# strasdat/ScaViSLAM

Hardware: AMD Instinct MI355X
Metric: stereo frames/sec + DWO Schur ms @ 50 KF / 20k pts (higher is better)
Workload: dtype u8/int32 (FAST, ZNSSD), f32+f64 (dense tracking), f64 (Schur); 1 GPU

## Files before the change

scavislam_amd/csrc/dense.hip:

```cpp
#include "common.h"
#include "lm6.h"
#include "seqsum.h"
#include <algorithm>

namespace {

constexpr int NSUM = 28;

struct Acc {
  double v[NSUM];
  long long n;
  __device__ __forceinline__ void zero() {
#pragma unroll
    for (int i = 0; i < NSUM; ++i) v[i] = 0;
    n = 0;
  }
};

template <class P>
__device__ __forceinline__ float interp32f(P m, int stride, float u, float v) {
  float x = floorf(u), y = floorf(v);
  float sx = u - x, sy = v - y;
  float wx0 = 1 - sx, wx1 = sx, wy0 = 1 - sy, wy1 = sy;
  int xi = (int)x, yi = (int)y;
  const P p = m + (unsigned)(yi * stride + xi);
  float v00 = p[0], v10 = p[1], v01 = p[stride], v11 = p[stride + 1];
  return (wx0 * wy0) * v00 + (wx0 * wy1) * v01 + (wx1 * wy0) * v10 + (wx1 * wy1) * v11;
}

struct LevelArgs {
  const float *cloud; const uint8_t *prev; const float *cur, *dx, *dy;
  int pstride, fstride;
  svs_cam cam;
  const uint8_t *cur8;
  int c8stride;
};

#define SVS_AS1 __attribute__((address_space(1)))
typedef float svs_f4 __attribute__((ext_vector_type(4)));
struct LevelArgsG {
  const SVS_AS1 float *cloud; const SVS_AS1 uint8_t *prev; const SVS_AS1 float *cur, *dx, *dy;
  int pstride, fstride;
  svs_cam cam;
  const SVS_AS1 uint8_t *cur8;
  int c8stride;
};
__device__ __forceinline__ float4 load_f4(const float *p) { return *reinterpret_cast<const float4 *>(p); }
__device__ __forceinline__ float4 load_f4(const SVS_AS1 float *p) { const svs_f4 v = *(const SVS_AS1 svs_f4 *)p; return make_float4(v.x, v.y, v.z, v.w); }
__device__ __forceinline__ uint32_t load_u32_unaligned(const uint8_t *p) { uint32_t w; __builtin_memcpy(&w, p, 4); return w; }
__device__ __forceinline__ uint32_t load_u32_unaligned(const SVS_AS1 uint8_t *p) {
  typedef uint32_t u32_unaligned __attribute__((aligned(1)));
  return *(const SVS_AS1 u32_unaligned *)p;
}

template <class P>
__device__ __forceinline__ void taps_u8(P img, int stride, float u, float v, float &ic, float &gx, float &gy) {
  const float sc = (float)(1. / 255.);
  const float x = floorf(u), y = floorf(v);
  const float sx = u - x, sy = v - y;
  const float wx0 = 1 - sx, wx1 = sx, wy0 = 1 - sy, wy1 = sy;
  const int xi = (int)x, yi = (int)y;
  float f[4][4];
  const unsigned o0 = (unsigned)((yi - 1) * stride + (xi - 1));
#pragma unroll
  for (int r = 0; r < 4; ++r) {
    const uint32_t w4 = load_u32_unaligned(img + (o0 + (unsigned)(r * stride)));
#pragma unroll
    for (int c = 0; c < 4; ++c) f[r][c] = (float)((w4 >> (8 * c)) & 0xff) * sc;
  }
  const float w00 = wx0 * wy0, w01 = wx0 * wy1, w10 = wx1 * wy0, w11 = wx1 * wy1;
  ic = w00 * f[1][1] + w01 * f[2][1] + w10 * f[1][2] + w11 * f[2][2];
  gx = w00 * (f[1][2] - f[1][0]) + w01 * (f[2][2] - f[2][0]) + w10 * (f[1][3] - f[1][1]) + w11 * (f[2][3] - f[2][1]);
  gy = w00 * (f[2][1] - f[0][1]) + w01 * (f[3][1] - f[1][1]) + w10 * (f[2][2] - f[0][2]) + w11 * (f[3][2] - f[1][2]);
}

struct SampleIn { float4 c4; uint8_t prev; };
template <class LA>
__device__ __forceinline__ SampleIn sample_load(const LA &L, int u, int v, int cw, bool in_range) {
  SampleIn s;
  s.c4 = in_range ? load_f4(L.cloud + 4u * (unsigned)(v * cw + u)) : make_float4(0.f, 0.f, 1.f, -1.f);
  s.prev = L.prev[(unsigned)(((in_range ? v : 0) * 4) * L.pstride + (in_range ? u : 0) * 4)];
  return s;
}
__device__ __forceinline__ double rcp_rn(double b) {
  double r = __builtin_amdgcn_rcp(b);
  double e = __builtin_fma(-b, r, 1.0);
  r = __builtin_fma(e, r, r);
  e = __builtin_fma(-b, r, 1.0);
  return __builtin_fma(e, r, r);
}
__device__ __forceinline__ double div_rn(double a, double b, double r) {
  const double q = a * r;
  return __builtin_fma(__builtin_fma(-q, b, a), r, q);
}

template <bool JAC, bool U8SRC = false, int TM = 0, class LA = LevelArgs>
__device__ __forceinline__ void sample_cpu_sem(const LA &L, const double *T, const SampleIn &in, bool in_range, Acc &a,
                                               const float *ip_lut = nullptr, float *term_out = nullptr) {
  const float4 c4 = in.c4;
  bool ok = in_range && (c4.w > 0);
  const double xp0 = c4.x, xp1 = c4.y, xp2 = c4.z;
  const double x = T[0] * xp0 + T[1] * xp1 + T[2] * xp2 + T[3];
  const double y = T[4] * xp0 + T[5] * xp1 + T[6] * xp2 + T[7];
  const double z = T[8] * xp0 + T[9] * xp1 + T[10] * xp2 + T[11];
  const double rz = rcp_rn(z);
  float uvx = (float)(L.cam.f * div_rn(x, z, rz) + L.cam.cx);
  float uvy = (float)(L.cam.f * div_rn(y, z, rz) + L.cam.cy);
  ok = ok && (fabsf(uvx) < 1e9f && fabsf(uvy) < 1e9f);
  const int ui = ok ? (int)uvx : 0, vi = ok ? (int)uvy : 0;
  ok = ok && (ui >= 2 && vi >= 2 && ui < L.cam.w - 2 && vi < L.cam.h - 2);
  if (!ok) { uvx = 2.f; uvy = 2.f; }
  const float ip = ip_lut ? ip_lut[in.prev] : (float)((1. / 255.) * in.prev);
  float ic, g8x = 0.f, g8y = 0.f;
  if (U8SRC) taps_u8(L.cur8, L.c8stride, uvx, uvy, ic, g8x, g8y);
  else ic = interp32f(L.cur, L.fstride, uvx, uvy);
  float res = ip - ic;
  res = fminf(fmaxf(res, -0.1f), 0.1f);
  if (!ok) res = 0.f;
  a.v[27] += (double)(res * res);
  if constexpr (TM != 0) *term_out = res * res;
  a.n += ok ? 1 : 0;
  if (JAC) {
    const float gx = ok ? (float)(0.5 * (U8SRC ? g8x : interp32f(L.dx, L.fstride, uvx, uvy))) : 0.f;
    const float gy = ok ? (float)(0.5 * (U8SRC ? g8y : interp32f(L.dy, L.fstride, uvx, uvy))) : 0.f;
    const double zs = ok ? z : 1.0, xs = ok ? x : 0.0, ys = ok ? y : 0.0;
    {
      const double f = L.cam.f, iz = ok ? rz : 1.0, iz2 = iz * iz, fx = f * iz, xz = xs * iz2 * f, yz = ys * iz2 * f;
      const double r0[6] = {-fx, 0, xz, xz * ys, -__builtin_fma(xz, xs, f), ys * fx};
      const double r1[6] = {0, -fx, yz, __builtin_fma(yz, ys, f), -(yz * xs), -(xs * fx)};
      double J[6];
      J[0] = gx * r0[0];
      J[1] = gy * r1[1];
#pragma unroll
      for (int k = 2; k < 6; ++k) J[k] = __builtin_fma(gx, r0[k], gy * r1[k]);
      int k = 0;
#pragma unroll
      for (int c = 0; c < 6; ++c)
#pragma unroll
        for (int r = 0; r <= c; ++r) { a.v[k] = __builtin_fma(J[r], J[c], a.v[k]); ++k; }
#pragma unroll
      for (int i = 0; i < 6; ++i) a.v[21 + i] = __builtin_fma(J[i], (double)res, a.v[21 + i]);
    }
  }
}

template <int NWAVES>
__device__ __forceinline__ void block_reduce(Acc &a, double (*s_part)[NSUM + 1], double *out_vals ) {
  const int lane = threadIdx.x & 63, wave = threadIdx.x >> 6;
  double x[32];
#pragma unroll
  for (int i = 0; i < NSUM; ++i) x[i] = a.v[i];
  x[NSUM] = (double)a.n;
#pragma unroll
  for (int i = NSUM + 1; i < 32; ++i) x[i] = 0.0;
#pragma unroll
  for (int step = 0; step < 5; ++step) {
    const int half = 16 >> step, bit = 1 << step;
    const bool up = (lane & bit) != 0;
#pragma unroll
    for (int k = 0; k < half; ++k) {
      const double send = up ? x[k] : x[k + half];
      const double keep = up ? x[k + half] : x[k];
      x[k] = keep + __shfl_xor(send, bit, 64);
    }
  }
  x[0] += __shfl_xor(x[0], 32, 64);
  const int idx = ((lane & 1) << 4) | ((lane & 2) << 2) | (lane & 4) | ((lane & 8) >> 2) | ((lane & 16) >> 4);
  if (lane < 32 && idx <= NSUM) s_part[wave][idx] = x[0];
  __syncthreads();
  if (threadIdx.x <= NSUM) {
    double s = 0;
    for (int w = 0; w < NWAVES; ++w) s += s_part[w][threadIdx.x];
    out_vals[threadIdx.x] = s;
  }
  __syncthreads();
}

template <bool JAC>
__global__ __launch_bounds__(256) void dense_pass_cpu_sem_kernel(LevelArgs L, size_t cloud_b, size_t prev_b, size_t f_b,
                                                                 const double *__restrict__ Tarr, double *__restrict__ partials) {
  __shared__ double s_part[4][NSUM + 1];
  __shared__ double s_out[NSUM + 1];
  const int slot = blockIdx.y;
  L.cloud += slot * cloud_b; L.prev += slot * prev_b; L.cur += slot * f_b; L.dx += slot * f_b; L.dy += slot * f_b;
  double T[12];
#pragma unroll
  for (int i = 0; i < 12; ++i) T[i] = Tarr[(size_t)slot * 12 + i];
  const int cw = L.cam.w / 4, ch = L.cam.h / 4, n = cw * ch;
  Acc a;
  a.zero();
  for (int i = blockIdx.x * 256 + threadIdx.x; i < n; i += gridDim.x * 256) sample_cpu_sem<JAC>(L, T, sample_load(L, i % cw, i / cw, cw, true), true, a);
  block_reduce<4>(a, s_part, s_out);
  if (threadIdx.x <= NSUM) partials[((size_t)slot * gridDim.x + blockIdx.x) * (NSUM + 1) + threadIdx.x] = s_out[threadIdx.x];
}

__global__ void dense_finalize_kernel(const double *__restrict__ partials, int nblocks, svs_dense_sums *__restrict__ out) {
  const int slot = blockIdx.x, t = threadIdx.x;
  if (t > NSUM) return;
  double s = 0;
  for (int b = 0; b < nblocks; ++b) s += partials[((size_t)slot * nblocks + b) * (NSUM + 1) + t];
  svs_dense_sums *o = &out[slot];
  if (t < 21) o->H[t] = s;
  else if (t < 27) o->b[t - 21] = s;
  else if (t == 27) o->chi2 = (double)(float)s;
  else o->n_valid = (long long)s;
}

struct TrackArgs {
  LevelArgs lv[3];
  size_t cloud_b[3], prev_b[3], f_b[3], c8_b[3];
  double *T_jac;
  svs_dense_lm_record *rec; int rec_cap; int32_t *n_rec;
};

constexpr int TRK_THREADS = 512;
constexpr int TRK_MINW_BIG = 4;
constexpr int TRK_UNROLL = 1;
constexpr bool TRK_T_SCALAR = true;

template <bool JAC, bool U8SRC, int TM = 0, class LA = LevelArgs>
__device__ __forceinline__ void track_pass(const LA &L, const double *T_in, double (*s_part)[NSUM + 1], double *s_out, const float *ip_lut,
                                           int first, int nwg, float *t_buf = nullptr) {
  const int cw = L.cam.w / 4, ch = L.cam.h / 4, n = cw * ch;
  double T[12];
#pragma unroll
  for (int i = 0; i < 12; ++i)
    T[i] = TRK_T_SCALAR ? __hiloint2double(__builtin_amdgcn_readfirstlane(__double2hiint(T_in[i])), __builtin_amdgcn_readfirstlane(__double2loint(T_in[i]))) : T_in[i];
  Acc a;
  a.zero();
  const int STEP = TRK_UNROLL * TRK_THREADS * nwg;
  const int su = STEP % cw, sv = STEP / cw;
  SampleIn nxt[TRK_UNROLL];
  int pu[TRK_UNROLL], pv[TRK_UNROLL];
#pragma unroll
  for (int q = 0; q < TRK_UNROLL; ++q) {
    const int j = first + q * TRK_THREADS * nwg;
    pu[q] = j % cw; pv[q] = j / cw;
    const bool in = pv[q] < ch;
    nxt[q] = sample_load(L, in ? pu[q] : 0, in ? pv[q] : 0, cw, in);
  }
  typedef __attribute__((address_space(1))) float *gptr_t;
  static_assert(TM == 0 || TRK_UNROLL == 1, "the deferred term store keeps one term per lane");
  float pend_t = 0.f;
  gptr_t pend_p = (gptr_t)t_buf + first - STEP;
  bool pend = false;
  auto flush = [&]() {
    if constexpr (TM == 1) { if (pend) *pend_p = pend_t; }
    if constexpr (TM == 2) { if (pend) __hip_atomic_store(pend_p, pend_t, __ATOMIC_RELAXED, __HIP_MEMORY_SCOPE_AGENT); }
  };
  for (int i = first; i < n; i += STEP) {
    if constexpr (TM != 0) { flush(); pend_p += STEP; pend = t_buf != nullptr; }
    SampleIn cur[TRK_UNROLL];
#pragma unroll
    for (int q = 0; q < TRK_UNROLL; ++q) {
      cur[q] = nxt[q];
      pu[q] += su; pv[q] += sv;
      if (pu[q] >= cw) { pu[q] -= cw; ++pv[q]; }
      const bool in = pv[q] < ch;
      nxt[q] = sample_load(L, in ? pu[q] : 0, in ? pv[q] : 0, cw, in);
    }
#pragma unroll
    for (int q = 0; q < TRK_UNROLL; ++q) {
      if constexpr (TM != 0) sample_cpu_sem<JAC, U8SRC, TM, LA>(L, T, cur[q], true, a, ip_lut, &pend_t);
      else sample_cpu_sem<JAC, U8SRC, 0, LA>(L, T, cur[q], i + q * TRK_THREADS * nwg < n, a, ip_lut);
    }
  }
  if constexpr (TM != 0) flush();
  block_reduce<TRK_THREADS / 64>(a, s_part, s_out);
}

struct PassArgs { LevelArgs L; double T[12]; float *t_buf; int wg, nwg; };
__shared__ PassArgs g_pa;
__shared__ double g_s_part[TRK_THREADS / 64][NSUM + 1];
__shared__ double g_s_out[NSUM + 1];
__shared__ float g_iplut[256];
__device__ __forceinline__ int uni_i32(int v) { return __builtin_amdgcn_readfirstlane(v); }
__device__ __forceinline__ double uni_f64(double v) { return __hiloint2double(__builtin_amdgcn_readfirstlane(__double2hiint(v)), __builtin_amdgcn_readfirstlane(__double2loint(v))); }
template <class T>
__device__ __forceinline__ T *uni_ptr(T *p) {
  const unsigned long long u = (unsigned long long)p;
  const unsigned lo = __builtin_amdgcn_readfirstlane((unsigned)u), hi = __builtin_amdgcn_readfirstlane((unsigned)(u >> 32));
  return (T *)(((unsigned long long)hi << 32) | lo);
}
template <bool U8SRC, int TM>
__device__ __forceinline__ void track_pass_from_lds() {
  LevelArgsG L;
  L.cloud = (const SVS_AS1 float *)uni_ptr(g_pa.L.cloud); L.prev = (const SVS_AS1 uint8_t *)uni_ptr(g_pa.L.prev);
  L.cur = (const SVS_AS1 float *)uni_ptr(g_pa.L.cur); L.dx = (const SVS_AS1 float *)uni_ptr(g_pa.L.dx); L.dy = (const SVS_AS1 float *)uni_ptr(g_pa.L.dy);
  L.cur8 = (const SVS_AS1 uint8_t *)uni_ptr(g_pa.L.cur8);
  L.pstride = uni_i32(g_pa.L.pstride); L.fstride = uni_i32(g_pa.L.fstride); L.c8stride = uni_i32(g_pa.L.c8stride);
  L.cam.f = uni_f64(g_pa.L.cam.f); L.cam.cx = uni_f64(g_pa.L.cam.cx); L.cam.cy = uni_f64(g_pa.L.cam.cy); L.cam.b = 0;
  L.cam.w = uni_i32(g_pa.L.cam.w); L.cam.h = uni_i32(g_pa.L.cam.h);
  const int nwg = uni_i32(g_pa.nwg), first = uni_i32(g_pa.wg) * TRK_THREADS + (int)threadIdx.x;
  track_pass<true, U8SRC, TM, LevelArgsG>(L, g_pa.T, g_s_part, g_s_out, g_iplut, first, nwg, uni_ptr(g_pa.t_buf));
}
template <bool U8SRC, int TM>
__device__ __noinline__ void track_pass_call() { track_pass_from_lds<U8SRC, TM>(); }

typedef const __attribute__((address_space(1))) float *svs_gptr_f32;
typedef const __attribute__((address_space(1))) svs_f4 *svs_gptr_f4;
template <bool COH, typename P>
__device__ __forceinline__ float seq_term_load(P p) {
  if constexpr (COH) return __hip_atomic_load(p, __ATOMIC_RELAXED, __HIP_MEMORY_SCOPE_AGENT); else return *p;
}
template <bool COH = false, typename P = const float *>
__device__ __forceinline__ float seq_sum_f32(P t, int n) {
  float acc = 0.f;
  const int lane = threadIdx.x & 63;
  for (int base = 0; base < n; base += 64) {
    const float v = base + lane < n ? seq_term_load<COH, P>(t + base + lane) : 0.f;
#pragma unroll
    for (int l = 0; l < 64; ++l) acc = acc + __builtin_bit_cast(float, __builtin_amdgcn_readlane(__builtin_bit_cast(int, v), l));
  }
  return acc;
}
__device__ __forceinline__ float seq_chi2_f32(const float *t, int n) {
  __shared__ float s_seq;
  __syncthreads();
  if (threadIdx.x < 64) { const float v = seq_sum_f32(t, n); if (threadIdx.x == 0) s_seq = v; }
  __syncthreads();
  return s_seq;
}

constexpr int SEQ_Q = TRK_THREADS >= 512 ? 10 : 13;
constexpr int SEQ_RUN_MAX = 4 * SEQ_Q;
constexpr int SEQ_STAGE_FLOATS = 48 * SEQ_RUN_MAX;
struct SeqShared {
  SvsSeqMap pref[TRK_THREADS];
  unsigned char eb[TRK_THREADS];
  short slot[TRK_THREADS];
  unsigned long long unsafe[TRK_THREADS / 64];
  double wave_P[TRK_THREADS / 64];
  int wave_c[TRK_THREADS / 64], wave_u[TRK_THREADS / 64];
  float stage[SEQ_STAGE_FLOATS];
  float result;
  int fell_back;
};
template <bool COH>
__device__ __forceinline__ void seq_load_run(svs_gptr_f32 p, int nq, svs_f4 (&v)[SEQ_Q]) {
  if constexpr (COH) {
    static_assert(SEQ_Q == 10 || SEQ_Q == 13, "the blocks below issue ten (+ three) loads");
    asm volatile("global_load_dwordx4 %0, %10, off sc1\n\t"
                 "global_load_dwordx4 %1, %10, off offset:16 sc1\n\t"
                 "global_load_dwordx4 %2, %10, off offset:32 sc1\n\t"
                 "global_load_dwordx4 %3, %10, off offset:48 sc1\n\t"
                 "global_load_dwordx4 %4, %10, off offset:64 sc1\n\t"
                 "global_load_dwordx4 %5, %10, off offset:80 sc1\n\t"
                 "global_load_dwordx4 %6, %10, off offset:96 sc1\n\t"
                 "global_load_dwordx4 %7, %10, off offset:112 sc1\n\t"
                 "global_load_dwordx4 %8, %10, off offset:128 sc1\n\t"
                 "global_load_dwordx4 %9, %10, off offset:144 sc1\n\t"
                 "s_waitcnt vmcnt(0)"
                 : "=&v"(v[0]), "=&v"(v[1]), "=&v"(v[2]), "=&v"(v[3]), "=&v"(v[4]), "=&v"(v[5]), "=&v"(v[6]), "=&v"(v[7]), "=&v"(v[8]), "=&v"(v[9])
                 : "v"(p)
                 : "memory");
    if constexpr (SEQ_Q == 13)
      asm volatile("global_load_dwordx4 %0, %3, off offset:160 sc1\n\t"
                   "global_load_dwordx4 %1, %3, off offset:176 sc1\n\t"
                   "global_load_dwordx4 %2, %3, off offset:192 sc1\n\t"
                   "s_waitcnt vmcnt(0)"
                   : "=&v"(v[SEQ_Q - 3]), "=&v"(v[SEQ_Q - 2]), "=&v"(v[SEQ_Q - 1])
                   : "v"(p)
                   : "memory");
  } else {
#pragma unroll
    for (int q = 0; q < SEQ_Q; ++q) v[q] = q < nq ? *reinterpret_cast<svs_gptr_f4>(p + 4 * q) : svs_f4{0.f, 0.f, 0.f, 0.f};
  }
}
__shared__ SeqShared g_seq_sh;
template <bool COH>
__device__ __noinline__ float exact_seq_sum_f32(const float *t_flat, int n) {
  SeqShared &sh = g_seq_sh;
  svs_gptr_f32 t = (svs_gptr_f32)t_flat;
  const int tid = threadIdx.x, lane = tid & 63, wave = tid >> 6;
  const int S = max(4, (div_up(n, TRK_THREADS) + 3) & ~3);
  if (S > SEQ_RUN_MAX) {
    __syncthreads();
    if (wave == 0) { const float v = seq_sum_f32<COH, svs_gptr_f32>(t, n); if (lane == 0) { sh.result = v; sh.fell_back = 1; } }
    __syncthreads();
    return sh.result;
  }
  const int nq = S / 4;
  const int j0 = min(n, tid * S), j1 = min(n, j0 + S);
  const bool empty = j0 >= j1;
  svs_f4 v[SEQ_Q];
  seq_load_run<COH>(t + (empty ? 0 : j0), nq, v);
  double ps = 0;
  int cnt = 0;
#pragma unroll
  for (int q = 0; q < SEQ_Q; ++q)
#pragma unroll
    for (int c = 0; c < 4; ++c) {
      if (!(q < nq && j0 + 4 * q + c < j1)) v[q][c] = 0.f;
      ps += (double)v[q][c];
      cnt += v[q][c] != 0.f ? 1 : 0;
    }
  double incl = ps;
  int cincl = cnt;
#pragma unroll
  for (int d = 1; d < 64; d <<= 1) {
    const double o = __shfl_up(incl, d, 64);
    const int oc = __shfl_up(cincl, d, 64);
    if (lane >= d) { incl += o; cincl += oc; }
  }
// ... 441 lines not shown
    int level;
    if (!resume) {
      track_pass_from_lds<U8SRC, TM>();
      if constexpr (MULTI) { all_workgroups(); if (s_failed) { failed = true; break; } }
      level = g_ts.level;
      const int phase = g_ts.phase, cur = g_ts.cur, n_rec = g_ts.n_rec;
      const int n_lvl = (A.lv[level].cam.w / 4) * (A.lv[level].cam.h / 4);
      if (phase == 0) {
        const double S = g_s_out[27];
        const float chi2 = (float)S;
        __syncthreads();
        if (tid < 27) g_sH[tid] = g_s_out[tid];
        if (tid == 0) {
          g_ts.S_old = S; g_ts.nv_old = (int)g_s_out[NSUM]; g_ts.chi2 = chi2; g_ts.seq_old_ok = 0; g_ts.seq_old = 0.f;
          ++g_ts.passes; ++g_ts.n_rec; g_ts.work16 += 16 >> (2 * level);
          if (A.rec && wg == 0 && n_rec < A.rec_cap) A.rec[(size_t)slot * A.rec_cap + n_rec] = svs_dense_lm_record{level, 2, chi2, chi2};
        }
      } else {
        const double S_old = g_ts.S_old, S_new = g_s_out[27];
        const int nv_old = g_ts.nv_old, nv_new = (int)g_s_out[NSUM];
        float seq_old = g_ts.seq_old;
        bool seq_old_ok = g_ts.seq_old_ok != 0;
        unsigned n_exact = 0;
        const TrkVerdict V = track_accept<MULTI>(G, slot, S_old, S_new, nv_old, nv_new, tb0, cur, n_lvl, true, wg, nwg, g_ts.chi2, seq_old, seq_old_ok, n_decisions, n_old_sums, n_exact);
        if (V.failed) { if (tid == 0) s_failed = true; failed = true; break; }
        const bool accept = V.accept;
        const float chi2 = V.chi2, new_chi2 = V.new_chi2;
        double mx = -1;
        for (int q = 0; q < 6; ++q) mx = fmax(mx, fabs(g_sx[q]));
        const int it = g_ts.it + 1;
        level_done = !accept || mx <= 1e-10 || it >= 15;
        __syncthreads();
        if (accept) {
          if (tid < 12) g_sT[tid] = g_sTn[tid];
          if (tid < 27) g_sH[tid] = g_s_out[tid];
        }
        if (tid == 0) {
          if (accept) { g_ts.S_old = S_new; g_ts.nv_old = nv_new; g_ts.cur = cur ^ 1; g_ts.chi2 = new_chi2; }
          g_ts.seq_old = seq_old; g_ts.seq_old_ok = seq_old_ok ? 1 : 0; g_ts.it = it; g_ts.n_exact += n_exact;
          ++g_ts.passes; ++g_ts.n_rec; g_ts.work16 += 16 >> (2 * level);
          if (A.rec && wg == 0 && n_rec < A.rec_cap) A.rec[(size_t)slot * A.rec_cap + n_rec] = svs_dense_lm_record{level, accept ? 1 : 0, chi2, new_chi2};
        }
        if constexpr (!MULTI) {
          if (!level_done && level == 0 && C.K >= 0 && it >= C.K) parked = true;
        }
      }
      __syncthreads();
      if (parked) break;
    } else {
      resume = false;
      level = g_ts.level;
    }
    if (level_done) {
      if (level == 0) break;
      if (tid == 0) enter_level(level - 1);
      if (tid >= 64 && tid < 76) g_pa.T[tid - 64] = g_sT[tid - 64];
    } else {
      if (tid >= 64 && tid < 76) g_sTj[level][tid - 64] = g_sT[tid - 64];
      if (tid < 64) track_solve_call();
      __syncthreads();
      if (tid < 12) g_pa.T[tid] = g_sTn[tid];
      if (tid == 12) { g_pa.t_buf = tb0 ? tb0 + (size_t)(g_ts.cur ^ 1) * G.terms_b : nullptr; g_ts.phase = 1; }
    }
    __syncthreads();
  }
  if constexpr (!MULTI) {
    if (parked) {
      TrkPark &P = C.park[slot];
      if (tid == 0) { P.ts = g_ts; C.list[atomicAdd(C.count, 1u)] = slot; }
      if (tid < 12) P.T[tid] = g_sT[tid];
      if (tid >= 64 && tid < 64 + 27) P.H[tid - 64] = g_sH[tid - 64];
      if (tid >= 128 && tid < 128 + 36) P.Tj[tid - 128] = g_sTj[(tid - 128) / 12][(tid - 128) % 12];
      return;
    }
  }
  if (wg != 0) return;
  if (failed) { if (tid == 0 && passes_out) passes_out[slot] = -1; return; }
  if (tid < 12) T_io[(size_t)slot * 12 + tid] = g_sT[tid];
  if (tid == 0 && passes_out) passes_out[slot] = g_ts.passes;
  if (tid == 0 && A.n_rec) A.n_rec[slot] = g_ts.n_rec;
  if (tid == 0 && G.work16) G.work16[slot] = g_ts.work16;
  if (A.T_jac && tid < 36) A.T_jac[(size_t)slot * 36 + tid] = g_sTj[tid / 12][tid % 12];
  if (tid == 0 && G.seq_stats && g_ts.n_exact) {
    atomicAdd(G.seq_stats, g_ts.n_exact);
    if (g_seq_sh.fell_back) atomicAdd(G.seq_stats + 1, 1u);
  }
}
template <bool U8SRC, bool BAL, int CONT>
__global__ __launch_bounds__(TRK_THREADS, TRK_MINW_BIG) void dense_track_batch_kernel(TrackArgs A, double *__restrict__ T_io, int *__restrict__ passes_out, TrackMulti G, TrackCont C) {
  if constexpr (CONT == 0) {
    int slot = blockIdx.x;
    if constexpr (BAL) {
      const int e = G.map[blockIdx.x];
      if (e < 0 || (e & 15) != 0) return;
      slot = e >> 4;
    }
    track_batch_stream<U8SRC, false>(A, T_io, passes_out, G, C, slot, 0, 1);
  } else {
    const int n_parked = (int)*C.count;
    for (int p = blockIdx.y; p < n_parked; p += gridDim.y) {
      track_batch_stream<U8SRC, true>(A, T_io, passes_out, G, C, C.list[p], blockIdx.x, CONT_MAX_NWG);
      __syncthreads();
    }
  }
}

template <bool U8SRC>
__global__ __launch_bounds__(256) void residual_image_cpu_sem_kernel(LevelArgs L, size_t cloud_b, size_t prev_b, size_t f_b, size_t c8_b,
                                                                     const double *__restrict__ Tarr, size_t T_b,
                                                                     float *__restrict__ rimg, size_t rimg_b) {
  const int slot = blockIdx.y;
  const int cw = L.cam.w / 4, ch = L.cam.h / 4;
  const int i = blockIdx.x * 256 + threadIdx.x;
  if (i >= cw * ch) return;
  L.cloud += slot * cloud_b; L.prev += slot * prev_b;
  if (U8SRC) L.cur8 += slot * c8_b; else L.cur += slot * f_b;
  double T[12];
#pragma unroll
  for (int k = 0; k < 12; ++k) T[k] = Tarr[(size_t)slot * T_b + k];
  const int u = i % cw, v = i / cw;
  const float4 c4 = reinterpret_cast<const float4 *>(L.cloud)[i];
  float4 o = make_float4(0.f, 1.f, 0.f, 1.f);
  if (c4.w > 0) {
    const double xp0 = c4.x, xp1 = c4.y, xp2 = c4.z;
    const double x = T[0] * xp0 + T[1] * xp1 + T[2] * xp2 + T[3];
    const double y = T[4] * xp0 + T[5] * xp1 + T[6] * xp2 + T[7];
    const double z = T[8] * xp0 + T[9] * xp1 + T[10] * xp2 + T[11];
    const float uvx = (float)(L.cam.f * (x / z) + L.cam.cx);
    const float uvy = (float)(L.cam.f * (y / z) + L.cam.cy);
    bool ok = fabsf(uvx) < 1e9f && fabsf(uvy) < 1e9f;
    const int ui = ok ? (int)uvx : 0, vi = ok ? (int)uvy : 0;
    ok = ok && (ui >= 2 && vi >= 2 && ui < L.cam.w - 2 && vi < L.cam.h - 2);
    o = make_float4(1.f, 0.f, 0.f, 1.f);
    if (ok) {
      const float ip = (float)((1. / 255.) * L.prev[(size_t)(v * 4) * L.pstride + u * 4]);
      float ic, gx, gy;
      if (U8SRC) taps_u8(L.cur8, L.c8stride, uvx, uvy, ic, gx, gy);
      else ic = interp32f(L.cur, L.fstride, uvx, uvy);
      float res = ip - ic;
      if (res > 0.1) res = 0.1;
      if (res < -0.1) res = -0.1;
      float g = 1 - 50.f * res * res;
      if (g < 0.f) g = 0.f;
      o = make_float4(g, g, g, 1.f);
    }
  }
  reinterpret_cast<float4 *>(rimg + slot * rimg_b)[i] = o;
}


}


static int ensure_scratch(svs_ctx *ctx, double **p, size_t count) {
  void *v = nullptr;
  const int rc = svs_ctx_scratch(ctx, count * sizeof(double), &v);
  *p = static_cast<double *>(v);
  return rc;
}


extern "C" int svs_dense_pass_cpu_sem(svs_ctx *ctx, const float *d_cloud, size_t cloud_bstride, const uint8_t *d_prev_u8,
                                      int pstride, size_t p_bstride, const float *d_cur, const float *d_dx,
                                      const float *d_dy, int fstride, size_t f_bstride, const svs_cam *cam,
                                      const double *d_T, int do_jac, svs_dense_sums *d_out, int batch) {
  SVS_REQUIRE(ctx, ctx && d_cloud && d_prev_u8 && d_cur && cam && d_T && d_out && batch >= 1);
  SVS_DEVICE(ctx);
  SVS_REQUIRE(ctx, !do_jac || (d_dx && d_dy));
  SVS_REQUIRE(ctx, cam->w % 4 == 0 && cam->h % 4 == 0);
  LevelArgs L{d_cloud, d_prev_u8, d_cur, d_dx, d_dy, pstride, fstride, *cam, nullptr, 0};
  int n = (cam->w / 4) * (cam->h / 4);
  int nblocks = std::min(div_up(n, 256), 256);
  double *part = nullptr;
  int rc = ensure_scratch(ctx, &part, (size_t)batch * nblocks * (NSUM + 1));
  if (rc) return rc;
  if (do_jac)
    hipLaunchKernelGGL(dense_pass_cpu_sem_kernel<true>, dim3(nblocks, batch), dim3(256), 0, ctx->stream, L, cloud_bstride, p_bstride, f_bstride, d_T, part);
  else
    hipLaunchKernelGGL(dense_pass_cpu_sem_kernel<false>, dim3(nblocks, batch), dim3(256), 0, ctx->stream, L, cloud_bstride, p_bstride, f_bstride, d_T, part);
  SVS_LAUNCH_CHECK(ctx);
  hipLaunchKernelGGL(dense_finalize_kernel, dim3(batch), dim3(64), 0, ctx->stream, part, nblocks, d_out);
  SVS_LAUNCH_CHECK(ctx);
  return SVS_OK;
}

namespace {
constexpr int BAL_MAX_STREAMS = 4096;
constexpr int ASSIGN_THREADS = 1024;
__global__ __launch_bounds__(ASSIGN_THREADS) void trk_assign_kernel(const svs_dense_lm_record *__restrict__ rec, int rec_cap, const int32_t *__restrict__ n_rec, int B, int slots, int x_max, int grid, float ratio, int *__restrict__ map,
                                                          unsigned char *__restrict__ nwg_of, const int *__restrict__ work16) {
  __shared__ __attribute__((aligned(16))) float s_w[BAL_MAX_STREAMS];
  __shared__ unsigned char s_n[BAL_MAX_STREAMS];
  __shared__ float s_red[ASSIGN_THREADS / 64];
  __shared__ int s_cnt[2];
  const int tid = threadIdx.x;
  int *s_wi = reinterpret_cast<int *>(s_w);
  for (int b = tid; b < B; b += ASSIGN_THREADS) s_wi[b] = 0;
  __syncthreads();
  if (work16) {
    for (int b = tid; b < B; b += ASSIGN_THREADS) s_wi[b] = work16[b];
  } else if (rec) {
    const int total = B * rec_cap;
    for (int base = tid; base < total; base += 8 * ASSIGN_THREADS) {
      int4 r[8];
#pragma unroll
      for (int u = 0; u < 8; ++u) { const int idx = base + u * ASSIGN_THREADS; r[u] = idx < total ? *reinterpret_cast<const int4 *>(rec + idx) : make_int4(3, 0, 0, 0); }
#pragma unroll
      for (int u = 0; u < 8; ++u) {
        const int idx = base + u * ASSIGN_THREADS;
        if (idx < total) {
          const int b = idx / rec_cap, i = idx - b * rec_cap, l = r[u].x;
          if (i < min(n_rec[b], rec_cap) && l >= 0 && l <= 2) atomicAdd(&s_wi[b], l == 0 ? 16 : (l == 1 ? 4 : 1));
        }
      }
    }
  }
  __syncthreads();
  float sum = 0.f;
  for (int b = tid; b < B; b += ASSIGN_THREADS) { const float w = (float)s_wi[b] * 0.0625f; s_w[b] = w; sum += w; }
  for (int o = 32; o > 0; o >>= 1) sum += __shfl_xor(sum, o, 64);
  if ((tid & 63) == 0) s_red[tid >> 6] = sum;
  __syncthreads();
  float mean = 0.f;
  for (int k = 0; k < ASSIGN_THREADS / 64; ++k) mean += s_red[k];
  mean /= (float)B;
  float M = ratio * mean;
  if (x_max == 0) {
    for (int b = tid; b < B; b += ASSIGN_THREADS) s_n[b] = 1;
    if (tid < 2) s_cnt[tid] = 0;
    __syncthreads();
  } else
  for (int round = 0; round < 24; ++round) {
    if (tid < 2) s_cnt[tid] = 0;
    __syncthreads();
    int extra = 0, multi = 0;
    for (int b = tid; b < B; b += ASSIGN_THREADS) {
      int n = 1;
      if (mean > 0.f) { n = (int)ceilf(s_w[b] / M); n = n < 1 ? 1 : (n > 4 ? 4 : n); }
      s_n[b] = (unsigned char)n;
      extra += n - 1; multi += n > 1 ? n : 0;
    }
    for (int o = 32; o > 0; o >>= 1) { extra += __shfl_xor(extra, o, 64); multi += __shfl_xor(multi, o, 64); }
    if ((tid & 63) == 0 && extra) { atomicAdd(&s_cnt[0], extra); atomicAdd(&s_cnt[1], multi); }
    __syncthreads();
    const bool fits = s_cnt[0] <= x_max && s_cnt[1] <= slots;
    __syncthreads();
    if (fits) break;
    M *= 1.08f;
    if (round == 23) { for (int b = tid; b < B; b += ASSIGN_THREADS) s_n[b] = 1; __syncthreads(); if (tid < 2) s_cnt[tid] = 0; __syncthreads(); }
  }
  const int n_multi_wgs = s_cnt[1];
  __syncthreads();
  int *s_key = reinterpret_cast<int *>(s_w);
  const int Bp = (B + 3) & ~3;
  for (int b = tid; b < Bp; b += ASSIGN_THREADS) {
    const int key = b < B && s_n[b] == 1 ? ((int)(s_w[b] * 16.f) << 12) | (4095 - b) : -1;
    s_key[b] = key;
  }
  for (int g = tid; g < grid; g += ASSIGN_THREADS) map[g] = -1;
  __syncthreads();
  for (int b = tid; b < B; b += ASSIGN_THREADS) {
    const int n = s_n[b];
    int pos = 0;
    if (n > 1) { for (int k = 0; k < b; ++k) pos += s_n[k] > 1 ? s_n[k] : 0; }
    else {
      const int mine = s_key[b];
      pos = n_multi_wgs;
      for (int k = 0; k < Bp; k += 4) {
        const int4 q = *reinterpret_cast<const int4 *>(s_key + k);
        pos += (q.x > mine) + (q.y > mine) + (q.z > mine) + (q.w > mine);
      }
    }
    for (int k = 0; k < n; ++k) map[pos + k] = (b << 4) | k;
    nwg_of[b] = (unsigned char)n;
  }
}

static int cont_setup(svs_ctx *ctx, int batch, TrackMulti &G, TrackCont &C) {
  const size_t n_part = (size_t)batch * 2 * CONT_MAX_NWG * 32, n_bar = (size_t)batch, n_bc = (size_t)batch * 16, n_cnt = 2, n_list = (size_t)batch / 2 + 1;
  const size_t n_park = ((size_t)batch * sizeof(TrkPark) + 7) / 8;
  double *scr = nullptr;
  const int rc = ensure_scratch(ctx, &scr, n_part + n_bar + n_bc + n_cnt + n_list + n_park);
  if (rc) return rc;
  G.part = scr;
  G.bar = reinterpret_cast<unsigned *>(scr + n_part);
  G.fail_off = batch;
  G.bcast = scr + n_part + n_bar;
  C.count = reinterpret_cast<unsigned *>(scr + n_part + n_bar + n_bc);
  C.list = reinterpret_cast<int *>(scr + n_part + n_bar + n_bc + n_cnt);
  C.park = reinterpret_cast<TrkPark *>(scr + n_part + n_bar + n_bc + n_cnt + n_list);
  C.K = ctx->trk_split; C.slots = ctx->trk_cont_slots > 0 ? ctx->trk_cont_slots : 2 * ctx->n_cu;
  SVS_HIP(ctx, hipMemsetAsync(G.bar, 0, sizeof(double) * (n_bar + n_bc + n_cnt), ctx->stream));
  return SVS_OK;
}
#define TRK_ARGS(...) __VA_ARGS__
#define TRK_LAUNCH(u8src, K, TAIL, grid, ...)                                                                              \
  do {                                                                                                                     \
    if (u8src) hipLaunchKernelGGL((K<true, TRK_ARGS TAIL>), grid, dim3(TRK_THREADS), 0, ctx->stream, __VA_ARGS__);         \
    else hipLaunchKernelGGL((K<false, TRK_ARGS TAIL>), grid, dim3(TRK_THREADS), 0, ctx->stream, __VA_ARGS__);              \
  } while (0)
template <bool BAL>
static int launch_batch_tracker(svs_ctx *ctx, const TrackArgs &A, bool u8src, double *d_T_io, int32_t *d_passes_out, int batch, int grid, TrackMulti G) {
  TrackCont C{nullptr, nullptr, nullptr, -1, 0};
  if (ctx->trk_split > 0) { const int rc = cont_setup(ctx, batch, G, C); if (rc) return rc; }
  TRK_LAUNCH(u8src, dense_track_batch_kernel, (BAL, 0), dim3(grid), A, d_T_io, d_passes_out, G, C);
  SVS_LAUNCH_CHECK(ctx);
  if (C.K < 0) return SVS_OK;
  const int groups = std::max(1, std::min(batch, C.slots / CONT_MAX_NWG));
  SvsSpinScope gate(ctx);
  if (gate.rc) return gate.rc;
  TRK_LAUNCH(u8src, dense_track_batch_kernel, (false, 1), dim3(CONT_MAX_NWG, groups), A, d_T_io, d_passes_out, G, C);
  SVS_LAUNCH_CHECK(ctx);
  return gate.leave();
}
struct BalState { int *map; unsigned char *nwg_of; double *flags; size_t n_flags; int grid, x_max; int *work16; };
BalState bal_state(void *state, int batch) {
  BalState S;
  S.x_max = batch / 2; S.grid = batch + S.x_max;
  char *p = static_cast<char *>(state);
  auto take = [&](size_t bytes) { char *q = p; p += (bytes + 255) & ~(size_t)255; return q; };
  S.map = reinterpret_cast<int *>(take(sizeof(int) * (size_t)S.grid));
  S.nwg_of = reinterpret_cast<unsigned char *>(take((size_t)batch));
  S.n_flags = (size_t)batch + (size_t)batch * 16;
  S.flags = reinterpret_cast<double *>(take(sizeof(double) * S.n_flags));
  S.work16 = reinterpret_cast<int *>(take(sizeof(int) * (size_t)batch));
  return S;
}
int bal_assign(svs_ctx *ctx, const BalState &S, int batch, const svs_dense_lm_record *rec, int rec_cap, const int32_t *n_rec, bool have_work = false) {
  const int x_max = ctx->trk_balance == 2 ? S.x_max : 0;
  const float ratio = 1.2f;
  hipLaunchKernelGGL(trk_assign_kernel, dim3(1), dim3(ASSIGN_THREADS), 0, ctx->stream, rec, rec_cap, n_rec, batch, 2 * ctx->n_cu, x_max, S.grid, ratio, S.map, S.nwg_of,
                     have_work ? S.work16 : nullptr);
  SVS_LAUNCH_CHECK(ctx);
  return SVS_OK;
}
int svs_dense_track_cpu_sem_balanced(svs_ctx *ctx, const TrackArgs &A, bool u8src, double *d_T_io, int32_t *d_passes_out, int batch, void *state, const TrackMulti &G0) {
  const BalState S = bal_state(state, batch);
  double *scratch = nullptr;
  int rc = ensure_scratch(ctx, &scratch, (size_t)batch * 2 * 4 * 32);
  if (rc) return rc;
  TrackMulti G = G0;
  G.part = scratch;
  G.bar = reinterpret_cast<unsigned *>(S.flags);
  G.fail_off = batch;
  G.bcast = S.flags + (size_t)batch;
  G.map = S.map; G.nwg_of = S.nwg_of;
  if (ctx->trk_balance == 2) {
    SVS_HIP(ctx, hipMemsetAsync(S.flags, 0, sizeof(double) * S.n_flags, ctx->stream));
    SvsSpinScope gate(ctx);
    if (gate.rc) return gate.rc;
    TRK_LAUNCH(u8src, dense_track_cpu_sem_kernel, (true, TRK_MINW_BIG, false, true), dim3(S.grid), A, d_T_io, d_passes_out, G);
    SVS_LAUNCH_CHECK(ctx);
    if (int grc = gate.leave()) return grc;
  } else if (ctx->trk_flat) {
    G.work16 = S.work16;
    if (int lrc = launch_batch_tracker<true>(ctx, A, u8src, d_T_io, d_passes_out, batch, S.grid, G)) return lrc;
    return bal_assign(ctx, S, batch, A.rec, A.rec_cap, A.n_rec, true);
  } else {
    TRK_LAUNCH(u8src, dense_track_cpu_sem_kernel, (false, TRK_MINW_BIG, false, true), dim3(S.grid), A, d_T_io, d_passes_out, G);
  }
  SVS_LAUNCH_CHECK(ctx);
  return bal_assign(ctx, S, batch, A.rec, A.rec_cap, A.n_rec);
}
}
const int *svs_dense_track_balance_order(svs_ctx *ctx, void *state, int batch) {
  return state && ctx->trk_balance == 1 ? bal_state(state, batch).map : nullptr;
}
size_t svs_dense_track_balance_bytes(int batch) {
  const uintptr_t base = 1 << 16;
  const BalState S = bal_state(reinterpret_cast<void *>(base), batch);
  return (size_t)(reinterpret_cast<uintptr_t>(S.work16) - base) + sizeof(int) * (size_t)batch + 256;
}
int svs_dense_track_balance_init(svs_ctx *ctx, void *state, int batch) {
  SVS_REQUIRE(ctx, ctx && state && batch >= 1 && batch <= BAL_MAX_STREAMS);
  SVS_DEVICE(ctx);
  SVS_HIP(ctx, hipMemsetAsync(state, 0, svs_dense_track_balance_bytes(batch), ctx->stream));
  return bal_assign(ctx, bal_state(state, batch), batch, nullptr, 0, nullptr);
}
extern "C" int svs_dense_track_cpu_sem(svs_ctx *ctx, const svs_dense_track_args *a, double *d_T_io, int32_t *d_passes_out,
                                       int batch) {
  return svs_dense_track_cpu_sem_work(ctx, a, d_T_io, d_passes_out, batch, nullptr);
}
int svs_dense_track_cpu_sem_work(svs_ctx *ctx, const svs_dense_track_args *a, double *d_T_io, int32_t *d_passes_out, int batch, void *d_bal_state) {
  SVS_REQUIRE(ctx, ctx && a && d_T_io && batch >= 1);
  SVS_DEVICE(ctx);
  TrackArgs A;
  const bool u8src = a->d_cur_u8[0] != nullptr;
  for (int l = 0; l < 3; ++l) {
    SVS_REQUIRE(ctx, a->d_cloud[l] && a->d_prev_u8[l]);
    SVS_REQUIRE(ctx, u8src ? a->d_cur_u8[l] != nullptr : (a->d_cur[l] && a->d_dx[l] && a->d_dy[l]));
    SVS_REQUIRE(ctx, a->cam_vec[l].w % 4 == 0 && a->cam_vec[l].h % 4 == 0);
    A.lv[l] = LevelArgs{a->d_cloud[l], a->d_prev_u8[l], a->d_cur[l], a->d_dx[l], a->d_dy[l], a->pstride[l], a->fstride[l], a->cam_vec[l],
                        a->d_cur_u8[l], a->c8stride[l]};
    A.cloud_b[l] = a->cloud_bstride[l]; A.prev_b[l] = a->p_bstride[l]; A.f_b[l] = a->f_bstride[l]; A.c8_b[l] = a->c8_bstride[l];
  }
  A.T_jac = a->d_T_jac_out;
  A.rec = a->d_record_out; A.rec_cap = a->d_record_out ? a->record_cap : 0; A.n_rec = a->d_n_record_out;
  SVS_REQUIRE(ctx, !a->d_record_out || a->record_cap > 0);
  int nwg = batch <= 16 ? 8 : (batch <= 32 ? 4 : 1);
  if (ctx->trk_nwg) nwg = ctx->trk_nwg;
  float *t_buf = nullptr; size_t t_b = 0;
  const bool seq_all = ctx->trk_seq_chi2 != 0, lazy = !seq_all && ctx->trk_lazy_chi2 != 0;
  float *terms = nullptr;
  if (seq_all || lazy) {
    if (seq_all) nwg = 1;
    t_b = (size_t)(a->cam_vec[0].w / 4) * (a->cam_vec[0].h / 4);
    if (lazy) t_b = ((t_b + 3) & ~(size_t)3) + 64;
    const size_t want = (size_t)batch * t_b * sizeof(float) * (lazy ? 2 : 1) + 256;
    if (ctx->seq_buf_bytes < want) {
      if (ctx->seq_buf) { SVS_HIP(ctx, hipStreamSynchronize(ctx->stream)); (void)hipFree(ctx->seq_buf); ctx->seq_buf = nullptr; ctx->seq_buf_bytes = 0; }
      SVS_HIP(ctx, hipMalloc(&ctx->seq_buf, want));
      ctx->seq_buf_bytes = want;
    }
    if (seq_all) t_buf = static_cast<float *>(ctx->seq_buf); else terms = static_cast<float *>(ctx->seq_buf);
    if (!ctx->seq_stats) {
      SVS_HIP(ctx, hipMalloc(&ctx->seq_stats, 256));
      SVS_HIP(ctx, hipMemsetAsync(ctx->seq_stats, 0, 256, ctx->stream));
    }
  }
  TrackMulti G{};
  G.terms = terms; G.terms_b = t_b; G.seq_stats = static_cast<unsigned *>(ctx->seq_stats); G.terms_only = ctx->trk_lazy_chi2 == 2;
  if (t_buf) {
    G.part = reinterpret_cast<double *>(t_buf); G.fail_off = (int)t_b;
    TRK_LAUNCH(u8src, dense_track_cpu_sem_kernel, (false, 2, true), dim3(batch), A, d_T_io, d_passes_out, G);
  } else if (nwg >= 2) {
    double *scratch = nullptr;
    const size_t n_part = (size_t)batch * 2 * nwg * 64;
    const size_t n_clear = (n_part + (size_t)batch + (size_t)batch * 16 + 7) & ~(size_t)7;
    int rc = ensure_scratch(ctx, &scratch, n_clear);
    if (rc) return rc;
    G.part = scratch;
    G.bar = reinterpret_cast<unsigned *>(scratch + n_part);
    G.fail_off = batch;
    G.bcast = scratch + n_part + (size_t)batch;
    SVS_HIP(ctx, hipMemsetAsync(scratch, 0, sizeof(double) * n_clear, ctx->stream));
    SvsSpinScope gate(ctx, nwg * batch);
    if (gate.rc) return gate.rc;
    TRK_LAUNCH(u8src, dense_track_cpu_sem_kernel, (true, 2), dim3(nwg, batch), A, d_T_io, d_passes_out, G);
    SVS_LAUNCH_CHECK(ctx);
    if (int grc = gate.leave()) return grc;
  } else if (d_bal_state && ctx->trk_balance && batch >= 2 * ctx->n_cu && batch <= BAL_MAX_STREAMS && A.rec && A.n_rec) {
    return svs_dense_track_cpu_sem_balanced(ctx, A, u8src, d_T_io, d_passes_out, batch, d_bal_state, G);
  } else if (((batch > ctx->n_cu && ctx->trk_regs != 1) || ctx->trk_regs == 2) && ctx->trk_flat) {
    if (int lrc = launch_batch_tracker<false>(ctx, A, u8src, d_T_io, d_passes_out, batch, batch, G)) return lrc;
  } else if ((batch > ctx->n_cu && ctx->trk_regs != 1) || ctx->trk_regs == 2) {
    TRK_LAUNCH(u8src, dense_track_cpu_sem_kernel, (false, TRK_MINW_BIG), dim3(batch), A, d_T_io, d_passes_out, G);
  } else {
    TRK_LAUNCH(u8src, dense_track_cpu_sem_kernel, (false, 2), dim3(batch), A, d_T_io, d_passes_out, G);
  }
  SVS_LAUNCH_CHECK(ctx);
  return SVS_OK;
}

namespace {
template <int HOW>
__global__ __launch_bounds__(TRK_THREADS) void seq_sum_probe_kernel(const float *__restrict__ t, int n, size_t bstride, float *__restrict__ out, int *__restrict__ fell_back) {
  if (threadIdx.x == 0) g_seq_sh.fell_back = 0;
  __syncthreads();
  const float *row = t + (size_t)blockIdx.x * bstride;
  float v;
  if constexpr (HOW == 2) v = seq_chi2_f32(row, n); else v = exact_seq_sum_f32<HOW == 1>(row, n);
  if (threadIdx.x == 0) { out[blockIdx.x] = v; if (fell_back) fell_back[blockIdx.x] = HOW == 2 ? 1 : g_seq_sh.fell_back; }
}
}
extern "C" int svs_dense_seq_sum_f32(svs_ctx *ctx, const float *d_terms, int n, size_t bstride, int batch, int how, float *d_out, int32_t *d_fell_back) {
  SVS_REQUIRE(ctx, ctx && d_terms && d_out && n >= 0 && batch >= 1 && how >= 0 && how <= 2);
  SVS_DEVICE(ctx);
  if (how == 0) hipLaunchKernelGGL(seq_sum_probe_kernel<0>, dim3(batch), dim3(TRK_THREADS), 0, ctx->stream, d_terms, n, bstride, d_out, d_fell_back);
  else if (how == 1) hipLaunchKernelGGL(seq_sum_probe_kernel<1>, dim3(batch), dim3(TRK_THREADS), 0, ctx->stream, d_terms, n, bstride, d_out, d_fell_back);
  else hipLaunchKernelGGL(seq_sum_probe_kernel<2>, dim3(batch), dim3(TRK_THREADS), 0, ctx->stream, d_terms, n, bstride, d_out, d_fell_back);
  SVS_LAUNCH_CHECK(ctx);
  return SVS_OK;
}

extern "C" int svs_dense_residual_image_cpu_sem(svs_ctx *ctx, const float *d_cloud, size_t cloud_bstride, const uint8_t *d_prev_u8,
                                                int pstride, size_t p_bstride, const float *d_cur, int fstride, size_t f_bstride,
                                                const uint8_t *d_cur_u8, int c8stride, size_t c8_bstride, const svs_cam *cam,
                                                const double *d_T, size_t T_bstride, float *d_res_img4, size_t res_bstride, int batch) {
  SVS_REQUIRE(ctx, ctx && d_cloud && d_prev_u8 && (d_cur || d_cur_u8) && cam && d_T && d_res_img4 && batch >= 1);
  SVS_DEVICE(ctx);
  SVS_REQUIRE(ctx, cam->w % 4 == 0 && cam->h % 4 == 0);
  LevelArgs L{d_cloud, d_prev_u8, d_cur, nullptr, nullptr, pstride, fstride, *cam, d_cur_u8, c8stride};
  const int n = (cam->w / 4) * (cam->h / 4);
  if (d_cur_u8)
    hipLaunchKernelGGL(residual_image_cpu_sem_kernel<true>, dim3(div_up(n, 256), batch), dim3(256), 0, ctx->stream, L, cloud_bstride, p_bstride,
                       f_bstride, c8_bstride, d_T, T_bstride, d_res_img4, res_bstride);
  else
    hipLaunchKernelGGL(residual_image_cpu_sem_kernel<false>, dim3(div_up(n, 256), batch), dim3(256), 0, ctx->stream, L, cloud_bstride, p_bstride,
                       f_bstride, c8_bstride, d_T, T_bstride, d_res_img4, res_bstride);
  SVS_LAUNCH_CHECK(ctx);
  return SVS_OK;
}
```

Measured before the change: 214,000 frames/s.

## Issue bilinear tap loads early via inline asm and overlap with Jacobian setup

Splits the u8 bilinear/gradient tap fetch into issue, wait and finish stages. The four row loads are emitted as inline global_load_dword using scalar base registers, and the Jacobian projection terms are computed between issue and wait to hide load latency. It also switches index arithmetic to 24-bit multiplies (guarded by new size checks), narrows the valid-count accumulator to int, and recomputes the deferred-store pointer from the loop index. The inline asm with a full vmcnt(0) wait and sched barriers limits compiler scheduling and could stall on other outstanding loads.

Result: faster. 217,300 frames/s (median of 6 runs) (+1.5%).

```diff
diff --git a/scavislam_amd/csrc/dense.hip b/scavislam_amd/csrc/dense.hip
--- a/scavislam_amd/csrc/dense.hip
+++ b/scavislam_amd/csrc/dense.hip
@@ -9,7 +9,7 @@
 
 struct Acc {
   double v[NSUM];
-  long long n;
+  int n;
   __device__ __forceinline__ void zero() {
 #pragma unroll
     for (int i = 0; i < NSUM; ++i) v[i] = 0;
@@ -53,33 +53,65 @@
   return *(const SVS_AS1 u32_unaligned *)p;
 }
 
-template <class P>
-__device__ __forceinline__ void taps_u8(P img, int stride, float u, float v, float &ic, float &gx, float &gy) {
+struct TapRows { uint32_t w[4]; };
+constexpr bool TRK_TAPS_ASM = true;
+template <bool ASM, class P>
+__device__ __forceinline__ void taps_u8_issue(P img, int stride, float u, float v, TapRows &t) {
+  const int xi = (int)floorf(u), yi = (int)floorf(v);
+  const unsigned o0 = __umul24(yi - 1, stride) + (unsigned)(xi - 1);
+  __builtin_amdgcn_sched_barrier(0);
+  if constexpr (ASM) {
+    const unsigned long long bv = (unsigned long long)img;
+    const unsigned long long b0 = ((unsigned long long)(unsigned)__builtin_amdgcn_readfirstlane((int)(bv >> 32)) << 32) | (unsigned)__builtin_amdgcn_readfirstlane((int)bv);
+    const unsigned long long rs = (unsigned long long)(unsigned)__builtin_amdgcn_readfirstlane(stride);
+    asm("global_load_dword %0, %4, %5\n\t"
+        "global_load_dword %1, %4, %6\n\t"
+        "global_load_dword %2, %4, %7\n\t"
+        "global_load_dword %3, %4, %8"
+        : "=&v"(t.w[0]), "=&v"(t.w[1]), "=&v"(t.w[2]), "=&v"(t.w[3])
+        : "v"(o0), "s"(b0), "s"(b0 + rs), "s"(b0 + 2 * rs), "s"(b0 + 3 * rs));
+  } else {
+#pragma unroll
+    for (int r = 0; r < 4; ++r) t.w[r] = load_u32_unaligned(img + (o0 + (unsigned)(r * stride)));
+  }
+  __builtin_amdgcn_sched_barrier(0);
+}
+template <bool ASM>
+__device__ __forceinline__ void taps_u8_wait(TapRows &t) {
+  __builtin_amdgcn_sched_barrier(0);
+  if constexpr (ASM) {
+    asm("s_waitcnt vmcnt(0)" : "+v"(t.w[0]), "+v"(t.w[1]), "+v"(t.w[2]), "+v"(t.w[3]));
+    __builtin_amdgcn_sched_barrier(0);
+  }
+}
+__device__ __forceinline__ void taps_u8_finish(const TapRows &t, float u, float v, float &ic, float &gx, float &gy) {
   const float sc = (float)(1. / 255.);
   const float x = floorf(u), y = floorf(v);
   const float sx = u - x, sy = v - y;
   const float wx0 = 1 - sx, wx1 = sx, wy0 = 1 - sy, wy1 = sy;
-  const int xi = (int)x, yi = (int)y;
   float f[4][4];
-  const unsigned o0 = (unsigned)((yi - 1) * stride + (xi - 1));
-#pragma unroll
-  for (int r = 0; r < 4; ++r) {
-    const uint32_t w4 = load_u32_unaligned(img + (o0 + (unsigned)(r * stride)));
-#pragma unroll
-    for (int c = 0; c < 4; ++c) f[r][c] = (float)((w4 >> (8 * c)) & 0xff) * sc;
-  }
+#pragma unroll
+  for (int r = 0; r < 4; ++r)
+#pragma unroll
+    for (int c = 0; c < 4; ++c) f[r][c] = (float)((t.w[r] >> (8 * c)) & 0xff) * sc;
   const float w00 = wx0 * wy0, w01 = wx0 * wy1, w10 = wx1 * wy0, w11 = wx1 * wy1;
   ic = w00 * f[1][1] + w01 * f[2][1] + w10 * f[1][2] + w11 * f[2][2];
   gx = w00 * (f[1][2] - f[1][0]) + w01 * (f[2][2] - f[2][0]) + w10 * (f[1][3] - f[1][1]) + w11 * (f[2][3] - f[2][1]);
   gy = w00 * (f[2][1] - f[0][1]) + w01 * (f[3][1] - f[1][1]) + w10 * (f[2][2] - f[0][2]) + w11 * (f[3][2] - f[1][2]);
 }
+template <class P>
+__device__ __forceinline__ void taps_u8(P img, int stride, float u, float v, float &ic, float &gx, float &gy) {
+  TapRows t;
+  taps_u8_issue<false>(img, stride, u, v, t);
+  taps_u8_finish(t, u, v, ic, gx, gy);
+}
 
 struct SampleIn { float4 c4; uint8_t prev; };
 template <class LA>
 __device__ __forceinline__ SampleIn sample_load(const LA &L, int u, int v, int cw, bool in_range) {
   SampleIn s;
-  s.c4 = in_range ? load_f4(L.cloud + 4u * (unsigned)(v * cw + u)) : make_float4(0.f, 0.f, 1.f, -1.f);
-  s.prev = L.prev[(unsigned)(((in_range ? v : 0) * 4) * L.pstride + (in_range ? u : 0) * 4)];
+  s.c4 = in_range ? load_f4(L.cloud + 4u * (__umul24(v, cw) + (unsigned)u)) : make_float4(0.f, 0.f, 1.f, -1.f);
+  s.prev = L.prev[__umul24((in_range ? v : 0) * 4, L.pstride) + (unsigned)((in_range ? u : 0) * 4)];
   return s;
 }
 __device__ __forceinline__ double rcp_rn(double b) {
@@ -111,9 +143,15 @@
   ok = ok && (ui >= 2 && vi >= 2 && ui < L.cam.w - 2 && vi < L.cam.h - 2);
   if (!ok) { uvx = 2.f; uvy = 2.f; }
   const float ip = ip_lut ? ip_lut[in.prev] : (float)((1. / 255.) * in.prev);
+  TapRows taps;
+  if constexpr (U8SRC) taps_u8_issue<TRK_TAPS_ASM>(L.cur8, L.c8stride, uvx, uvy, taps);
+  const double zs = ok ? z : 1.0, xs = ok ? x : 0.0, ys = ok ? y : 0.0;
+  const double f = L.cam.f, iz = ok ? rz : 1.0, iz2 = iz * iz, fx = f * iz, xz = xs * iz2 * f, yz = ys * iz2 * f;
   float ic, g8x = 0.f, g8y = 0.f;
-  if (U8SRC) taps_u8(L.cur8, L.c8stride, uvx, uvy, ic, g8x, g8y);
+  if constexpr (U8SRC) { taps_u8_wait<TRK_TAPS_ASM>(taps); taps_u8_finish(taps, uvx, uvy, ic, g8x, g8y); }
   else ic = interp32f(L.cur, L.fstride, uvx, uvy);
+  const double r0[6] = {-fx, 0, xz, xz * ys, -__builtin_fma(xz, xs, f), ys * fx};
+  const double r1[6] = {0, -fx, yz, __builtin_fma(yz, ys, f), -(yz * xs), -(xs * fx)};
   float res = ip - ic;
   res = fminf(fmaxf(res, -0.1f), 0.1f);
   if (!ok) res = 0.f;
@@ -123,11 +161,7 @@
   if (JAC) {
     const float gx = ok ? (float)(0.5 * (U8SRC ? g8x : interp32f(L.dx, L.fstride, uvx, uvy))) : 0.f;
     const float gy = ok ? (float)(0.5 * (U8SRC ? g8y : interp32f(L.dy, L.fstride, uvx, uvy))) : 0.f;
-    const double zs = ok ? z : 1.0, xs = ok ? x : 0.0, ys = ok ? y : 0.0;
     {
-      const double f = L.cam.f, iz = ok ? rz : 1.0, iz2 = iz * iz, fx = f * iz, xz = xs * iz2 * f, yz = ys * iz2 * f;
-      const double r0[6] = {-fx, 0, xz, xz * ys, -__builtin_fma(xz, xs, f), ys * fx};
-      const double r1[6] = {0, -fx, yz, __builtin_fma(yz, ys, f), -(yz * xs), -(xs * fx)};
       double J[6];
       J[0] = gx * r0[0];
       J[1] = gy * r1[1];
@@ -219,8 +253,9 @@
 constexpr bool TRK_T_SCALAR = true;
 
 template <bool JAC, bool U8SRC, int TM = 0, class LA = LevelArgs>
-__device__ __forceinline__ void track_pass(const LA &L, const double *T_in, double (*s_part)[NSUM + 1], double *s_out, const float *ip_lut,
+__device__ __forceinline__ void track_pass(const LA &L_in, const double *T_in, double (*s_part)[NSUM + 1], double *s_out, const float *ip_lut,
                                            int first, int nwg, float *t_buf = nullptr) {
+  const LA L = L_in;
   const int cw = L.cam.w / 4, ch = L.cam.h / 4, n = cw * ch;
   double T[12];
 #pragma unroll
@@ -240,16 +275,19 @@
     nxt[q] = sample_load(L, in ? pu[q] : 0, in ? pv[q] : 0, cw, in);
   }
   typedef __attribute__((address_space(1))) float *gptr_t;
+  typedef __attribute__((address_space(1))) char *gptr_c;
   static_assert(TM == 0 || TRK_UNROLL == 1, "the deferred term store keeps one term per lane");
   float pend_t = 0.f;
-  gptr_t pend_p = (gptr_t)t_buf + first - STEP;
+  const gptr_c pend_base = (gptr_c)(gptr_t)t_buf - 4 * (long)STEP;
   bool pend = false;
+  int i = first;
   auto flush = [&]() {
+    const gptr_t pend_p = (gptr_t)(pend_base + 4u * (unsigned)i);
     if constexpr (TM == 1) { if (pend) *pend_p = pend_t; }
     if constexpr (TM == 2) { if (pend) __hip_atomic_store(pend_p, pend_t, __ATOMIC_RELAXED, __HIP_MEMORY_SCOPE_AGENT); }
   };
-  for (int i = first; i < n; i += STEP) {
-    if constexpr (TM != 0) { flush(); pend_p += STEP; pend = t_buf != nullptr; }
+  for (; i < n; i += STEP) {
+    if constexpr (TM != 0) { flush(); pend = t_buf != nullptr; }
     SampleIn cur[TRK_UNROLL];
 #pragma unroll
     for (int q = 0; q < TRK_UNROLL; ++q) {
@@ -997,6 +1035,10 @@
 }
 
 
+static bool offsets_fit_24(const svs_cam &cam, int pstride, int c8stride) {
+  const int lim = 1 << 24;
+  return cam.w > 0 && cam.h > 0 && cam.w < lim && cam.h < lim && pstride >= 0 && pstride < lim && c8stride >= 0 && c8stride < lim;
+}
 static int ensure_scratch(svs_ctx *ctx, double **p, size_t count) {
   void *v = nullptr;
   const int rc = svs_ctx_scratch(ctx, count * sizeof(double), &v);
@@ -1013,6 +1055,7 @@
   SVS_DEVICE(ctx);
   SVS_REQUIRE(ctx, !do_jac || (d_dx && d_dy));
   SVS_REQUIRE(ctx, cam->w % 4 == 0 && cam->h % 4 == 0);
+  SVS_REQUIRE(ctx, offsets_fit_24(*cam, pstride, 0));
   LevelArgs L{d_cloud, d_prev_u8, d_cur, d_dx, d_dy, pstride, fstride, *cam, nullptr, 0};
   int n = (cam->w / 4) * (cam->h / 4);
   int nblocks = std::min(div_up(n, 256), 256);
@@ -1235,6 +1278,7 @@
     SVS_REQUIRE(ctx, a->d_cloud[l] && a->d_prev_u8[l]);
     SVS_REQUIRE(ctx, u8src ? a->d_cur_u8[l] != nullptr : (a->d_cur[l] && a->d_dx[l] && a->d_dy[l]));
     SVS_REQUIRE(ctx, a->cam_vec[l].w % 4 == 0 && a->cam_vec[l].h % 4 == 0);
+    SVS_REQUIRE(ctx, offsets_fit_24(a->cam_vec[l], a->pstride[l], u8src ? a->c8stride[l] : 0));
     A.lv[l] = LevelArgs{a->d_cloud[l], a->d_prev_u8[l], a->d_cur[l], a->d_dx[l], a->d_dy[l], a->pstride[l], a->fstride[l], a->cam_vec[l],
                         a->d_cur_u8[l], a->c8stride[l]};
     A.cloud_b[l] = a->cloud_bstride[l]; A.prev_b[l] = a->p_bstride[l]; A.f_b[l] = a->f_bstride[l]; A.c8_b[l] = a->c8_bstride[l];
@@ -1325,6 +1369,7 @@
   SVS_REQUIRE(ctx, ctx && d_cloud && d_prev_u8 && (d_cur || d_cur_u8) && cam && d_T && d_res_img4 && batch >= 1);
   SVS_DEVICE(ctx);
   SVS_REQUIRE(ctx, cam->w % 4 == 0 && cam->h % 4 == 0);
+  SVS_REQUIRE(ctx, offsets_fit_24(*cam, pstride, d_cur_u8 ? c8stride : 0));
   LevelArgs L{d_cloud, d_prev_u8, d_cur, nullptr, nullptr, pstride, fstride, *cam, d_cur_u8, c8stride};
   const int n = (cam->w / 4) * (cam->h / 4);
   if (d_cur_u8)
```
